# waleedbinkhalid74/cnn-gp

Measured on AMD Instinct MI355X. Metric: kernel entries/s (N×M pairs) + full-Kxx build+solve wall-clock, MNIST 28×28, higher is better.
Workload: dtype f64; 1 GPU; mnist_paper_convnet_gp Kxx 4096x4096, tiles 1024; n=4096, tile=1024, parallelism=tiles-dp1

## Files before the change

### cnn-gp_amd/cnn_gp/_native.py

```python
from __future__ import annotations

import ctypes
import os
import threading

_HERE = os.path.dirname(os.path.abspath(__file__))
LIB_PATH = os.environ.get("CNNGP_LIB",
                          os.path.join(os.path.dirname(_HERE), "lib", "libcnngp.so"))

CGP_ABI_VERSION = 12
CGP_FLAG_EXACT_RELU = 1
CGP_FLAG_GENERIC_CONV = 2
CGP_FLAG_NET_DUAL = 4
CGP_PRE_NONE, CGP_PRE_RELU, CGP_PRE_MOMENTS = 0, 1, 2
CGP_POST_NONE, CGP_POST_RELU = 0, 1
CGP_NET_CONV, CGP_NET_RELU, CGP_NET_MOMENTS, CGP_NET_LINEAR = 0, 1, 2, 3
CGP_NET_LOAD, CGP_NET_STORE = 4, 5
CGP_NET_CODE_HS_CLEAN = 0x100
CGP_NET_CODE_SUM = 0x200
CGP_NET_CODE_FROM_SUM = 0x400
CGP_NET_CODE_GEOMETRY = 0xff
CGP_VAR_MOMENTS, CGP_VAR_CONV, CGP_VAR_HALF, CGP_VAR_SUM = 0, 1, 2, 3

_vp = ctypes.c_void_p
_i64 = ctypes.c_int64
_i32 = ctypes.c_int32
_f64 = ctypes.c_double


class ConvArgs(ctypes.Structure):
    _fields_ = [
        ("in_", _vp), ("in_y", _vp), ("out", _vp), ("addend", _vp),
        ("pre_xx", _vp), ("pre_yy", _vp), ("post_xx", _vp), ("post_yy", _vp),
        ("nmaps", _i64), ("n1", _i64), ("n2", _i64),
        ("h", _i32), ("w", _i32), ("ho", _i32), ("wo", _i32),
        ("taps", _i32), ("offset", _i32), ("stride", _i32), ("dilation", _i32),
        ("channels", _i32), ("pre", _i32), ("post", _i32), ("same", _i32), ("diag", _i32),
        ("maps_per_block", _i32), ("flags", _i32), ("reserved", _i32),
        ("weight", _f64), ("bias", _f64),
    ]


class ReluArgs(ctypes.Structure):
    _fields_ = [
        ("xy", _vp), ("out", _vp), ("addend", _vp), ("xx", _vp), ("yy", _vp),
        ("nmaps", _i64), ("n1", _i64), ("n2", _i64),
        ("hw", _i32), ("same", _i32), ("diag", _i32), ("flags", _i32),
    ]


class ReluNtkArgs(ctypes.Structure):
    _fields_ = [
        ("xy", _vp), ("theta", _vp), ("out_xy", _vp), ("out_theta", _vp),
        ("xx", _vp), ("yy", _vp),
        ("nmaps", _i64), ("n1", _i64), ("n2", _i64),
# ... 23 lines not shown


class VarArgs(ctypes.Structure):
    _fields_ = [
        ("x", _vp), ("y", _vp), ("out", _vp), ("ops", _vp),
        ("n1", _i64), ("n2", _i64), ("store_total", _i64),
        ("nops", _i32), ("channels", _i32), ("h", _i32), ("w", _i32),
        ("lds_elems", _i32), ("scratch", _i32),
    ]


class NetArgs(ctypes.Structure):
    _fields_ = [
        ("x", _vp), ("y", _vp), ("out", _vp), ("kdiag", _vp), ("ops", _vp),
        ("n1", _i64), ("n2", _i64), ("ldo", _i64),
        ("nops", _i32), ("channels", _i32), ("h", _i32), ("w", _i32),
        ("same", _i32), ("final_slot", _i32), ("hs", _i32), ("lds_elems", _i32),
        ("flags", _i32), ("pairs", _i32), ("unit_begin", _i64), ("unit_end", _i64),
        ("final_stage", _i32), ("program", _i32), ("part", _i32),
    ]


def make_fastdiv(d: int):
    s = 0
    while (1 << s) < d:
        s += 1
    m = (((1 << 32) * ((1 << s) - d)) // d + 1) & 0xFFFFFFFF
    return m, s


SIGNATURES = {
    "cgp_abi_version": (_i32, []),
    "cgp_net_xvar_scale": (ctypes.c_double, []),
    "cgp_last_error": (ctypes.c_char_p, []),
    "cgp_conv_args_size": (ctypes.c_size_t, []),
    "cgp_relu_args_size": (ctypes.c_size_t, []),
    "cgp_device_count": (_i32, []),
    "cgp_selftest": (_i32, []),
    "cgp_moments_xy_f64": (_i32, [_vp, _vp, _i64, _i64, _i32, _i32, _i32, _vp, _vp]),
    "cgp_moments_xy_f32": (_i32, [_vp, _vp, _i64, _i64, _i32, _i32, _i32, _vp, _vp]),
    "cgp_moments_var_f64": (_i32, [_vp, _vp, _i64, _i64, _i32, _i32, _vp, _vp, _vp]),
    "cgp_moments_var_f32": (_i32, [_vp, _vp, _i64, _i64, _i32, _i32, _vp, _vp, _vp]),
    "cgp_conv_f64": (_i32, [ctypes.POINTER(ConvArgs), _vp]),
    "cgp_conv_f32": (_i32, [ctypes.POINTER(ConvArgs), _vp]),
    "cgp_relu_f64": (_i32, [ctypes.POINTER(ReluArgs), _vp]),
    "cgp_relu_f32": (_i32, [ctypes.POINTER(ReluArgs), _vp]),
    "cgp_relu_ntk_args_size": (ctypes.c_size_t, []),
    "cgp_relu_ntk_f64": (_i32, [ctypes.POINTER(ReluNtkArgs), _vp]),
    "cgp_relu_ntk_f32": (_i32, [ctypes.POINTER(ReluNtkArgs), _vp]),
    "cgp_var_relu_f64": (_i32, [_vp, _vp, _i64, _i64, _i32, _i32, _vp, _vp, _vp]),
    "cgp_var_relu_f32": (_i32, [_vp, _vp, _i64, _i64, _i32, _i32, _vp, _vp, _vp]),
    "cgp_axpby_f64": (_i32, [_f64, _vp, _f64, _vp, _vp, _i64, _vp]),
    "cgp_axpby_f32": (_i32, [_f64, _vp, _f64, _vp, _vp, _i64, _vp]),
    "cgp_scale_batch_f64": (_i32, [_i32, _vp, _vp, _vp, _f64, _vp]),
    "cgp_cast_f32_f64": (_i32, [_vp, _vp, _i64, _vp]),
    "cgp_transpose_f64": (_i32, [_vp, _i64, _i64, _vp, _vp]),
    "cgp_chol_solve_f64": (_i32, [_vp, _i64, _i64, _vp, _i64, _i64, _f64,
                                  ctypes.POINTER(_i64), _vp]),
    "cgp_chol_last_phases": (_i32, [_vp, ctypes.POINTER(_f64)]),
    "cgp_chol_solve_f64_timed": (_i32, [_vp, _i64, _i64, _vp, _i64, _i64, _f64,
                                        ctypes.POINTER(_i64), ctypes.POINTER(_f64), _vp]),
    "cgp_gemm_f64": (_i32, [_vp, _vp, _vp, _i64, _i64, _i64, _vp]),
    "cgp_sym_mirror_f64": (_i32, [_vp, _i64, _i64, _vp, _vp]),
    "cgp_sym_residual_f64": (_i32, [_vp, _i64, _i64, _vp, _vp, _vp, _i64, _i64, _vp, _vp]),
    "cgp_argmax_rows_f64": (_i32, [_vp, _i64, _i64, _vp, _vp]),
    "cgp_pred_var_f64": (_i32, [_vp, _i64, _i64, _vp, _i64, _i64, _vp, _vp, _vp]),
    "cgp_net_geometry": (_i32, [_i32] * 7),
    "cgp_net_hs_elems": (_i32, [_i32]),
    "cgp_net_supertile": (_i32, []),
    "cgp_net_units": (_i32, [_i32]),
    "cgp_net_resolution": (_i32, [_i32, _i32]),
    "cgp_net_op_size": (ctypes.c_size_t, []),
    "cgp_net_args_size": (ctypes.c_size_t, []),
    "cgp_net_occupancy": (_i32, [_i32, _i32, _i32, _i32]),
    "cgp_net_program": (_i32, [_vp, _i32, _i32, _i32, _i32, _i32]),
    "cgp_net_validate": (_i32, [_vp, _i32, _i32]),
    "cgp_net_static_lds": (_i32, []),
    "cgp_net_f64": (_i32, [ctypes.POINTER(NetArgs), _vp]),
    "cgp_net_f32": (_i32, [ctypes.POINTER(NetArgs), _vp]),
    "cgp_var_op_size": (ctypes.c_size_t, []),
    "cgp_var_args_size": (ctypes.c_size_t, []),
    "cgp_var_chain_f64": (_i32, [ctypes.POINTER(VarArgs), _vp]),
    "cgp_var_chain_f32": (_i32, [ctypes.POINTER(VarArgs), _vp]),
}

_lib = None
_lib_err = None
# ... 54 lines not shown
```

### cnn-gp_amd/cnn_gp/kernels.py

```python
from __future__ import annotations

import os
from typing import Optional

import numpy as np
import torch
import torch.nn as nn

from . import _native as N
from .program import Plan

VAR_CHAIN = os.environ.get("CGP_VAR_CHAIN", "1") != "0"

__all__ = ("NNGPKernel", "Conv2d", "ReLU", "Sequential", "Mixture", "Sum", "resnet_block")


def _stream_handle(device):
    return torch.cuda.current_stream(device).cuda_stream


def _to_device(t: torch.Tensor, device) -> torch.Tensor:
    if t.device != device:
        t = t.to(device, non_blocking=True)
    return t.contiguous()


class _ImageVariances:

    __slots__ = ("images", "var", "qvar", "key")

    def __init__(self, images, var, qvar, key):
        self.images, self.var, self.qvar, self.key = images, var, qvar, key

    def __len__(self):
        return len(self.images)


_GENERATION = [0]


class NNGPKernel(nn.Module):

    def __setattr__(self, name, value):
        _GENERATION[0] += 1
        super().__setattr__(name, value)

    def __delattr__(self, name):
        _GENERATION[0] += 1
        super().__delattr__(name)

    def add_module(self, name, module):
        _GENERATION[0] += 1
        super().add_module(name, module)

    def register_buffer(self, name, tensor, persistent=True):
        _GENERATION[0] += 1
        super().register_buffer(name, tensor, persistent)

    def _apply(self, fn, *args, **kwargs):
        _GENERATION[0] += 1
        out = super()._apply(fn, *args, **kwargs)
        _GENERATION[0] += 1
        return out

    def _plan(self, h: int, w: int) -> Plan:
# ... 146 lines not shown
                                                        N.ptr(var0[:n1]), N.ptr(var0[n1:]),
                                                        stream), "cgp_moments_var")
        var = plan.run_variances(var0[:n1], var0[n1:], n1, n2, same, stream,
                                 need=plan.ntk_need_var())
        nmaps = n1 if diag else n1 * n2
        xy0 = torch.empty((nmaps, h, w), dtype=x.dtype, device=x.device)
        N.check(getattr(lib, f"cgp_moments_xy_{sfx}")(N.ptr(x), N.ptr(y), n1, n2, c, h * w,
                                                       int(diag), N.ptr(xy0), stream),
                "cgp_moments_xy")
        k, th = plan.run_pairs_ntk(xy0, var, n1, n2, same, diag, stream)
        if th is None:
            th = torch.zeros_like(k)
        elif th is k:
            th = k.clone()
        shape = (n1,) if diag else (n1, n2)
        return k.view(shape), th.view(shape)

    def _run(self, x, y, same, diag, stream):
        n1, c, h, w = x.shape
        n2 = y.shape[0]
        plan = self._plan(h, w)
        sfx = Plan._sfx(x.dtype)
        lib = N.load()
        if diag and same and VAR_CHAIN and self._net_plan(plan, x.element_size()) is not None:
            fused = plan.run_variances_fused(x, x, n1, n1, True, stream, {plan.vf})
            if fused is not None:
                return fused[0][plan.vf][0].reshape(n1)
        net = None if diag else self._net_plan(plan, x.element_size())
        if net is not None and VAR_CHAIN:
            rec = net.tile_recipe(plan, x, y, n1, n2, same, plan.flags, stream)
            if rec is not None:
                return rec.run(x, y, stream)
            fused = plan.run_variances_fused(x, y, n1, n2, same, stream, net.need_var,
                                             net.quarter_vars(x.dtype, plan.flags),
                                             views=False)
            if fused is not None:
                var, qvar = fused
                return net.run(x, y, var, n1, n2, same, stream, plan.flags, qvar=qvar)
        var0 = torch.empty((n1 + n2, h, w), dtype=x.dtype, device=x.device)
        N.check(getattr(lib, f"cgp_moments_var_{sfx}")(N.ptr(x), N.ptr(y), n1, n2, c, h * w,
                                                        N.ptr(var0[:n1]), N.ptr(var0[n1:]),
                                                        stream), "cgp_moments_var")
        if net is not None:
            var = plan.run_variances(var0[:n1], var0[n1:], n1, n2, same, stream,
                                     need=net.need_var)
            return net.run(x, y, var, n1, n2, same, stream, plan.flags)
        var = plan.run_variances(var0[:n1], var0[n1:], n1, n2, same, stream)
        xy0 = None
        if not plan.moments_fused:
            nmaps = n1 if diag else n1 * n2
            xy0 = torch.empty((nmaps, h, w), dtype=x.dtype, device=x.device)
            N.check(getattr(lib, f"cgp_moments_xy_{sfx}")(N.ptr(x), N.ptr(y), n1, n2, c, h * w,
                                                           int(diag), N.ptr(xy0), stream),
                    "cgp_moments_xy")
        out = plan.run_pairs(x, y, xy0, var, n1, n2, same, diag, stream)
        if plan.final_hw != (1, 1):
            raise RuntimeError(f"the model's output is {plan.final_hw[0]}x{plan.final_hw[1]}"
                               " per pair, not 1x1: add a final Conv2d covering the map")
        return out.view(n1) if diag else out.view(n1, n2)


    def image_variances(self, x: torch.Tensor, max_bytes: Optional[int] = None):
        if x.device.type != "cuda" or x.dtype not in (torch.float32, torch.float64) or \
                x.dim() != 4 or not VAR_CHAIN:
            return None
        n, _, h, w = x.shape
        plan = self._plan(h, w)
        net = self._net_plan(plan, x.element_size())
        if net is None:
            return None
        quarter = net.quarter_vars(x.dtype, plan.flags)
        chain = plan._var_chain(set(net.need_var), set(quarter) & set(net.need_var), x.device)
        if chain is None:
            return None
        size = n * (chain["total"] + chain["qtotal"]) * x.element_size()
        if max_bytes is None:
            max_bytes = torch.cuda.mem_get_info(x.device)[0] // 4
        if size > max_bytes:
            return None
        x = x.contiguous()
        with torch.cuda.device(x.device):
            fused = plan.run_variances_fused(x, x, n, n, True, _stream_handle(x.device),
                                             net.need_var, quarter)
        if fused is None:
            return None
        var, qvar = fused
        return _ImageVariances(x, {v: xx for v, (xx, _) in var.items()}, dict(qvar),
                               (h, w, x.dtype, plan.flags, self._weights_version()))

    def tile_from_variances(self, vx: "_ImageVariances", i0: int, i1: int,
                            vy: "_ImageVariances", j0: int, j1: int, same: bool,
                            out: Optional[torch.Tensor] = None) -> torch.Tensor:
        if vx.key != vy.key:
            raise ValueError("tile_from_variances: the two image sets were prepared for "
                             "different shapes, dtypes or ReLU modes")
        if same and (vx is not vy or (i0, i1) != (j0, j1)):
            raise ValueError("a diagonal tile takes the same rows of one image set")
        if not (0 <= i0 < i1 <= len(vx) and 0 <= j0 < j1 <= len(vy)):
            raise ValueError(f"tile rows [{i0}, {i1}) x cols [{j0}, {j1}) outside the image "
                             f"sets ({len(vx)}, {len(vy)})")
        h, w, dtype, flags, wver = vx.key
        plan = self._plan(h, w)
        if plan.flags != flags:
            raise ValueError("tile_from_variances: the model's ReLU mode changed since "
                             "image_variances")
        if self._weights_version() != wver:
            raise ValueError("tile_from_variances: a Conv2d weight buffer changed since "
                             "image_variances (bind the image sets again)")
        net = self._net_plan(plan, torch.empty((), dtype=dtype).element_size())
        x, y = vx.images[i0:i1], vy.images[j0:j1]
        var = {v: (m[i0:i1], vy.var[v][j0:j1]) for v, m in vx.var.items()}
        qvar = {v: q[i0:i1] for v, q in vx.qvar.items()}
        with torch.cuda.device(x.device):
            return net.run(x, y, var, i1 - i0, j1 - j0, same, _stream_handle(x.device),
                           flags, out=out, qvar=qvar or None)

    def layers(self):
        return 0


class Conv2d(NNGPKernel):

    def __init__(self, kernel_size, stride=1, padding="same", dilation=1,
                 var_weight=1., var_bias=0., in_channel_multiplier=1,
                 out_channel_multiplier=1):
        super().__init__()
        self.kernel_size = kernel_size
        self.stride = stride
        self.dilation = dilation
        self.var_weight = var_weight
        self.var_bias = var_bias
        self.kernel_has_row_of_zeros = False
        self._padding_arg = padding
        if padding == "same":
            self.padding = dilation * (kernel_size // 2)
            self.kernel_has_row_of_zeros = kernel_size % 2 == 0
        else:
            self.padding = padding
        side = kernel_size + 1 if self.kernel_has_row_of_zeros else kernel_size
        kernel = torch.ones(1, 1, side, side)
        if self.kernel_has_row_of_zeros:
            kernel[:, :, 0, :] = 0.
            kernel[:, :, :, 0] = 0.
        self.register_buffer("kernel", kernel * (self.var_weight / self.kernel_size ** 2))
        self.in_channel_multiplier = in_channel_multiplier
        self.out_channel_multiplier = out_channel_multiplier

    def layers(self):
# ... 86 lines not shown
```

### cnn-gp_amd/cnn_gp/netplan.py

```python
from __future__ import annotations

import collections
import ctypes
import dataclasses
import os
import threading
from typing import Optional

import torch

from . import _native as N
from .program import fuse

ALIGN = 2

TIMING = None

USE_PROGRAMS = os.environ.get("CGP_NET_PROGRAMS", "1") != "0"
FUSE_REDUCE = os.environ.get("CGP_NET_FUSE_REDUCE", "1") != "0"
MAX_LDS_BYTES = 160 * 1024
SMALL_STATE_BYTES = 512 << 20
RECIPE_MAX_BYTES = int(os.environ.get("CGP_RECIPE_MAX_MB", "512")) << 20
RECIPE_SLOTS = 32
RECIPE_TOTAL_BYTES = 4 << 30
# ... 520 lines not shown
            o.dst2 = f.get("dst2", -1)
            o.zero_halo = _zero_code(f.get("zero")) | (_zero_code(f.get("zero2")) << 16)
            if var is None:
                continue
            if v is not None:
                vx, vy = var[v]
                o.var_x, o.var_y = vx.data_ptr(), vy.data_ptr()
            if "var2" in f:
                vx, vy = var[f["var2"]]
                o.var2_x, o.var2_y = vx.data_ptr(), vy.data_ptr()
            if f.get("state") == "in":
                o.var_x = state_in.data_ptr()
            elif f.get("state") == "out":
                o.var_x = state_out.data_ptr()
        return arr

    def chunk_units(self, itemsize: int, units: int, device=None) -> int:
        stride = max(max(st.load_stride, st.store_stride) for st in self.stages)
        chunk = CHUNK_BYTES // (stride * itemsize)
        per_unit = sum(st.load_stride for st in self.stages[1:]) * itemsize
        if device is not None and torch.device(device).type == "cuda" and \
                min(chunk, units) * per_unit > SMALL_STATE_BYTES:
            free = torch.cuda.mem_get_info(device)[0]
            chunk = min(chunk, int(free * STATE_FREE_FRAC) // max(1, per_unit))
        return min(max(64, chunk // 64 * 64), units)

    @staticmethod
    def units(n1: int, n2: int, same: bool) -> int:
        st = N.load().cgp_net_supertile()
        nbi, nbj = -(-n1 // st), -(-n2 // st)
        return (nbi * (nbi + 1) // 2 if same else nbi * nbj) * st * st

    def prepare(self, x, y, var, n1: int, n2: int, same: bool, flags: int = 0,
                out: Optional[torch.Tensor] = None, qvar: Optional[dict] = None):
        sfx = "f64" if x.dtype == torch.float64 else "f32"
        if out is None:
            out = torch.empty((n1, n2), dtype=x.dtype, device=x.device)
        if out.shape != (n1, n2) or out.stride(1) != 1 or out.dtype != x.dtype:
            raise ValueError("out must be an [n1, n2] row-major view of the input dtype")
        units = self.units(n1, n2, same)
        multi = len(self.stages) > 1
        chunk = units
        states = [None] * (len(self.stages) + 1)
        if multi:
            chunk = self.chunk_units(x.element_size(), units, x.device)
            for b in range(1, len(self.stages)):
                states[b] = torch.empty((chunk * self.stages[b].load_stride,),
                                        dtype=x.dtype, device=x.device)
        lib = N.load()
        fn = getattr(lib, f"cgp_net_{sfx}")
        launches = []
        keep = []
        quarters = []
        used = self.quarter_vars(x.dtype, flags)
        if used:
            var = dict(var)
            for v in sorted(used):
                vx, vy = var[v]
                if qvar is not None:
                    var[v] = (qvar[v], vy)
                    continue
                q = torch.empty_like(vx)
                quarters.append((vx, q))
                keep.append(q)
                var[v] = (q, vy)
        tmpls = [self._ops_template(sidx, st, flags, x.element_size())
                 for sidx, st in enumerate(self.stages)]
        offs = [0]
        for t in tmpls:
            offs.append(offs[-1] + len(t[0]))
        host = torch.empty((offs[-1],), dtype=torch.uint8, pin_memory=True)
        hb = host.numpy()
        for sidx, (tmpl, slots, what, _) in enumerate(tmpls):
            ptrs = [var[w[0]][w[1]].data_ptr() if isinstance(w, tuple) else
                    (states[sidx] if w == "in" else states[sidx + 1]).data_ptr()
                    for w in what]
            blk = hb[offs[sidx]:offs[sidx + 1]]
            blk[:] = tmpl
            blk.view("<u8")[slots] = ptrs
        ops_dev = host.to(x.device, non_blocking=True)
        keep.append(ops_dev)
        for sidx, st in enumerate(self.stages):
            program = tmpls[sidx][3]
            a = N.NetArgs()
            a.x, a.y, a.out = x.data_ptr(), y.data_ptr(), out.data_ptr()
            if same:
                a.kdiag = var[self.plan.vf][0].data_ptr()
            a.ops = ops_dev.data_ptr() + offs[sidx]
            a.n1, a.n2, a.ldo = n1, n2, out.stride(0)
            a.nops, a.channels, a.h, a.w = st.n_ops, x.shape[1], x.shape[2], x.shape[3]
            a.same, a.final_slot, a.hs, a.lds_elems = int(same), st.final_slot, 0, st.lds_elems
            a.part = st.part
            a.flags = flags | (N.CGP_FLAG_NET_DUAL if st.dual else 0)
            a.pairs = st.pairs
            a.final_stage = int(st.final)
            a.program = program
            launches.append(a)

        pairs = n1 * (n1 - 1) // 2 if same else n1 * n2

        if quarters:
            xscale = lib.cgp_net_xvar_scale()
            nq = len(quarters)
            q_src = (ctypes.c_void_p * nq)(*[N.ptr(s_) for s_, _ in quarters])
            q_dst = (ctypes.c_void_p * nq)(*[N.ptr(q_) for _, q_ in quarters])
            q_n = (ctypes.c_int64 * nq)(*[s_.numel() for s_, _ in quarters])

        def run_all(stream):
            if quarters:
                N.call("cgp_scale_batch_f64", nq, q_src, q_dst, q_n, xscale, stream)
            for u0 in range(0, units, chunk):
                u1 = min(units, u0 + chunk)
                for a in launches:
                    if multi:
                        a.unit_begin, a.unit_end = u0, u1
                    N.check(fn(ctypes.byref(a), stream), "cgp_net")

        def launch(stream, keep=keep, states=states):
            cur = torch.cuda.current_stream(x.device)
            if stream and stream != cur.cuda_stream:
                ext = torch.cuda.ExternalStream(stream, device=x.device)
                ext.wait_stream(cur)
                for t in keep + [s for s in states if s is not None]:
                    t.record_stream(ext)
            if TIMING is not None:
                st_ = torch.cuda.ExternalStream(stream) if stream else torch.cuda.current_stream()
                e0 = torch.cuda.Event(enable_timing=True)
                e1 = torch.cuda.Event(enable_timing=True)
                e0.record(st_)
                run_all(stream)
                e1.record(st_)
                TIMING.append((e0, e1, pairs))
            else:
                run_all(stream)

        launch.args = launches
        launch.states = states
        return launch, out

    def quarter_vars(self, dtype, flags: int = 0) -> set:
        if dtype != torch.float64 or flags & N.CGP_FLAG_EXACT_RELU:
            return set()
        used = self.__dict__.get("_quarter_used")
        if used is None:
            used = set()
            for st in self.stages:
                used |= {v for _, v in st.records if v is not None}
                used |= {f["var2"] for f, _ in st.records if "var2" in f}
            self.__dict__["_quarter_used"] = used
        return set(used)

    def tile_recipe(self, plan, x, y, n1: int, n2: int, same: bool, flags: int, stream):
        if RECIPE_MAX_BYTES <= 0:
            return None
        key = (n1, n2, bool(same), tuple(x.shape[1:]), x.dtype, x.device, flags, stream)
        lock = self.__dict__.setdefault("_recipe_lock", threading.Lock())
        with lock:
            cache = self.__dict__.setdefault("_recipes", collections.OrderedDict())
            if key in cache:
                cache.move_to_end(key)
                return cache[key]
            rec = TileRecipe.build(self, plan, x, y, n1, n2, same, flags, stream)
            if rec is None:
                return None
            cache[key] = rec
            while len(cache) > RECIPE_SLOTS or (
                    len(cache) > 1 and sum(r.nbytes for r in cache.values()) > RECIPE_TOTAL_BYTES):
                cache.popitem(last=False)
            return rec

    def run(self, x, y, var, n1: int, n2: int, same: bool, stream, flags: int = 0,
            out: Optional[torch.Tensor] = None, qvar: Optional[dict] = None):
        launch, out = self.prepare(x, y, var, n1, n2, same, flags, out, qvar)
        launch(stream)
        return out


class TileRecipe:

    def __init__(self):
        self.lock = threading.Lock()

    @classmethod
    def build(cls, net, plan, x, y, n1, n2, same, flags, stream):
        from .program import DevPtr
        need = set(net.need_var)
        quarter = net.quarter_vars(x.dtype, flags) & need
        chain = plan._var_chain(need, quarter, x.device)
        if chain is None or chain["lds"] * x.element_size() > 64 * 1024 or \
                x.shape[2] * x.shape[3] > 1024:
            return None
        m2 = 0 if same else n2
        n = n1 + m2
        item = x.element_size()
        vbytes = (n * chain["total"] + n1 * chain["qtotal"]) * item
        units = net.units(n1, n2, same)
        sbytes = sum(units * st.load_stride for st in net.stages[1:]) * item
        if vbytes + sbytes > RECIPE_MAX_BYTES:
            return None
        r = cls()
        r.nbytes = vbytes + sbytes
        r.shape = (n1, n2, tuple(x.shape[1:]), x.dtype, x.device)
        r.same = bool(same)
        r.vbuf = torch.empty((vbytes // item,), dtype=x.dtype, device=x.device)
        a = N.VarArgs()
        a.out, a.ops = r.vbuf.data_ptr(), chain["ops"].data_ptr()
        a.n1, a.n2, a.store_total = n1, m2, chain["total"]
        a.nops, a.channels, a.h, a.w = chain["nops"], x.shape[1], x.shape[2], x.shape[3]
        a.lds_elems, a.scratch = chain["lds"], chain["scratch"]
        r.va = a
        r.var_fn = getattr(N.load(), f"cgp_var_chain_{plan._sfx(x.dtype)}")
        r.chain_ops = chain["ops"]
        var, qvar = {}, {}
        shapes = plan.prog.shapes
        for v, off in chain["store"].items():
            ho, wo = shapes[v]
            px = DevPtr(r.vbuf, n * off * item)
            var[v] = (px, px if same else DevPtr(r.vbuf, (n * off + n1 * ho * wo) * item))
        for v, off in chain["qstore"].items():
            qvar[v] = DevPtr(r.vbuf, (n * chain["total"] + n1 * off) * item)
        out = torch.empty((n1, n2), dtype=x.dtype, device=x.device)
        r.launch, _ = net.prepare(x, y, var, n1, n2, same, flags, out, qvar or None)
        r.args = r.launch.args
        return r

    def run(self, x, y, stream):
        n1, n2, _, _, _ = self.shape
        out = torch.empty((n1, n2), dtype=x.dtype, device=x.device)
        xp, yp, op = x.data_ptr(), y.data_ptr(), out.data_ptr()
        with self.lock:
            self.va.x, self.va.y = xp, yp
            N.check(self.var_fn(self.va, stream), "cgp_var_chain")
            for a in self.args:
                a.x, a.y, a.out, a.ldo = xp, yp, op, n2
# ... 3 lines not shown
```

### cnn-gp_amd/csrc/cgp_common.h

```cpp
#pragma once

#include <hip/hip_runtime.h>

#include <string>

#include "cnngp.h"
#include "relu_poly.h"

namespace cgp {

int fail(int code, const char* fmt, ...);
int check_launch(const char* what);
int device_cus();
inline hipStream_t as_stream(void* s) { return reinterpret_cast<hipStream_t>(s); }
inline hipError_t stream_device(hipStream_t s, int* dev) {
    if (s == nullptr) return hipGetDevice(dev);
    hipDevice_t d = 0;
    const hipError_t e = hipStreamGetDevice(s, &d);
    if (e == hipSuccess) *dev = (int)d;
    return e;
}

#define CGP_HIP(call)                                                                  \
    do {                                                                               \
// ... 69 lines not shown
__device__ __forceinline__ float rsqrt_fast(float t) { return __builtin_amdgcn_rsqf(t); }
__device__ __forceinline__ double sqrt_fast(double x) {
    const double r = __builtin_amdgcn_rsq(x);
    const double s0 = x * r;
    return __builtin_fma(0.5 * r, __builtin_fma(-s0, s0, x), s0);
}
__device__ __forceinline__ float sqrt_fast(float x) { return x * __builtin_amdgcn_rsqf(x); }
__device__ __forceinline__ double relu_poly(double x) {
    double r = kReluPolyD[kReluPolyDegD];
#pragma unroll
    for (int k = kReluPolyDegD - 1; k >= 0; --k) r = __builtin_fma(r, x, kReluPolyD[k]);
    return r;
}
__device__ __forceinline__ float relu_poly(float x) {
    float r = kReluPolyF[kReluPolyDegF];
#pragma unroll
    for (int k = kReluPolyDegF - 1; k >= 0; --k) r = __builtin_fmaf(r, x, kReluPolyF[k]);
    return r;
}
__device__ __forceinline__ double fmin_t(double a, double b) { return __builtin_fmin(a, b); }
__device__ __forceinline__ float fmin_t(float a, float b) { return __builtin_fminf(a, b); }
__device__ __forceinline__ double fmax_t(double a, double b) { return __builtin_fmax(a, b); }
__device__ __forceinline__ float fmax_t(float a, float b) { return __builtin_fmaxf(a, b); }
__device__ __forceinline__ double fabs_t(double a) { return __builtin_fabs(a); }
__device__ __forceinline__ float fabs_t(float a) { return __builtin_fabsf(a); }
__device__ __forceinline__ double fma_t(double a, double b, double c) {
    return __builtin_fma(a, b, c);
}
__device__ __forceinline__ float fma_t(float a, float b, float c) {
    return __builtin_fmaf(a, b, c);
}

constexpr double kXVarScale = 0.0625;
constexpr double kPolyQ = 0.125;
constexpr double poly_q(int k) {
    double v = kReluPolyD[k] * kPolyQ;
    for (int n = 0; n < k; ++n) v *= 0.25;
    return v;
}
struct PolyCoef {
    double c[kReluPolyDegD + 1];
};
constexpr PolyCoef poly_coef(bool quartered) {
    PolyCoef t{};
    for (int k = 0; k <= kReluPolyDegD; ++k) t.c[k] = quartered ? poly_q(k) : kReluPolyD[k];
    return t;
}
static __constant__ PolyCoef kReluPolyTabD = poly_coef(false);
static __constant__ PolyCoef kReluPolyTabDq = poly_coef(true);

template <int D>
struct AdaptCoef {
    double c[D + 1];
};
template <int D>
constexpr AdaptCoef<D> adapt_coef(const double (&p)[D + 1]) {
    AdaptCoef<D> t{};
    for (int k = 0; k <= D; ++k) {
        double v = p[k] * kPolyQ;
        for (int n = 0; n < k; ++n) v *= 0.25;
        t.c[k] = v;
    }
    return t;
}
static __constant__ AdaptCoef<kReluAdaptDeg0> kReluAdaptTab0 = adapt_coef<kReluAdaptDeg0>(kReluAdaptP0);
static __constant__ AdaptCoef<kReluAdaptDeg1> kReluAdaptTab1 = adapt_coef<kReluAdaptDeg1>(kReluAdaptP1);
static __constant__ AdaptCoef<kReluAdaptDeg2> kReluAdaptTab2 = adapt_coef<kReluAdaptDeg2>(kReluAdaptP2);
// ... 66 lines not shown
    }
#pragma unroll
    for (int r = 0; r < R; ++r)
        c[r] = __builtin_fma(sx[r], p[r], (c[r] + __builtin_fabs(c[r])) * 0.25);
}
template <int R, int D>
__device__ __forceinline__ void horner_q(double (&p)[R], const double (&u)[R], ConstD t) {
#pragma unroll
    for (int r = 0; r < R; ++r) p[r] = fma_sc(t[D], u[r], t[D - 1]);
#pragma unroll
    for (int k = D - 2; k >= 0; --k) {
        const double ck = t[k];
#pragma unroll
        for (int r = 0; r < R; ++r) p[r] = fma_sc(p[r], u[r], ck);
    }
}
#ifndef CGP_RELU_VOTE_HI
#define CGP_RELU_VOTE_HI 1
#endif
__device__ __forceinline__ unsigned vote_hi(double v) {
    return (unsigned)(__builtin_bit_cast(unsigned long long, v) >> 32);
}
template <int R>
__device__ __forceinline__ unsigned vote_hi_max(const double (&u)[R]) {
    unsigned m = vote_hi(u[0]);
#pragma unroll
    for (int r = 1; r < R; ++r) m = m > vote_hi(u[r]) ? m : vote_hi(u[r]);
    return m;
}
template <int R, bool QIN, int AD = 0>
__device__ __forceinline__ void relu_q_n(double (&c)[R], const double (&v1q)[R],
                                         const double (&v2)[R], const PolyTab& tab,
                                         unsigned long long seg = ~0ull) {
    double y[R], st[R], sx[R], u[R], p[R];
#pragma unroll
    for (int r = 0; r < R; ++r) {
        if constexpr (!QIN) c[r] *= 0.25;
        const double T = __builtin_fma(v1q[r], v2[r], kXVarScale * K<double>::tiny);
        const double r0 = __builtin_amdgcn_rsq(T);
        const double m = T * r0;
        const double k = __builtin_fma(-m, r0, 3.0);
        y[r] = r0 * k;
        st[r] = m * k;
    }
#pragma unroll
    for (int r = 0; r < R; ++r) {
        u[r] = __builtin_fmax(__builtin_fma(-__builtin_fabs(c[r]), y[r], 2.0), 2.0 - 2.0 * kRhoMax);
        const double h = __builtin_amdgcn_rsq(u[r]);
        const double m = u[r] * h;
        const double sq4 = m * __builtin_fma(-m, h, 3.0);
        sx[r] = (st[r] * u[r]) * sq4;
    }
    if constexpr (AD == 2) {
        const unsigned long long ex = __builtin_amdgcn_read_exec() & seg;
        auto all_seg = [&](bool pred) { return (__ballot(pred) & seg) == ex; };
#if CGP_RELU_VOTE_HI
        const unsigned hm = vote_hi_max<R>(u);
        if (all_seg(hm < vote_hi(4.0 * kReluAdaptX0))) {
            horner_q<R, kReluAdaptDeg0>(p, u, tab.a0);
        } else if (all_seg(hm < vote_hi(4.0 * kReluAdaptX1))) {
            horner_q<R, kReluAdaptDeg1>(p, u, tab.a1);
        } else if (all_seg(hm < vote_hi(4.0 * kReluAdaptX2))) {
#else
        double um = u[0];
#pragma unroll
        for (int r = 1; r < R; ++r) um = __builtin_fmax(um, u[r]);
        if (all_seg(um <= 4.0 * kReluAdaptX0)) {
            horner_q<R, kReluAdaptDeg0>(p, u, tab.a0);
        } else if (all_seg(um <= 4.0 * kReluAdaptX1)) {
            horner_q<R, kReluAdaptDeg1>(p, u, tab.a1);
        } else if (all_seg(um <= 4.0 * kReluAdaptX2)) {
#endif
            horner_q<R, kReluAdaptDeg2>(p, u, tab.a2);
        } else {
            horner_q<R, kReluPolyDegD>(p, u, tab.dq);
        }
    } else if constexpr (AD == 1) {
#if CGP_RELU_VOTE_HI
        const unsigned hm = vote_hi_max<R>(u);
        if (__all(hm < vote_hi(4.0 * kReluAdaptX0))) {
            horner_q<R, kReluAdaptDeg0>(p, u, tab.a0);
        } else if (__all(hm < vote_hi(4.0 * kReluAdaptX1))) {
            horner_q<R, kReluAdaptDeg1>(p, u, tab.a1);
        } else if (__all(hm < vote_hi(4.0 * kReluAdaptX2))) {
#else
// ... 141 lines not shown
```

### cnn-gp_amd/csrc/cnngp.hip

```cpp

#include <hip/hip_runtime.h>
#include <rocblas/rocblas.h>
#include <rocsolver/rocsolver.h>

#include <cstdarg>
#include <cstdio>
#include <algorithm>
#include <cstring>
#include <map>
#include <mutex>
#include <string>
#include <vector>

#include "cnngp.h"
#include "cgp_common.h"

namespace cgp {


thread_local std::string g_last_error;

int fail(int code, const char* fmt, ...) {
    char buf[512];
    va_list ap;
// ... 643 lines not shown
        const int px = (int)(f - img * hw);
        const T* src = (is_x ? x : y) + (size_t)img * c * hw + px;
        T acc = src[0] * src[0];
        for (int k = 1; k < c; ++k) acc += src[(size_t)k * hw] * src[(size_t)k * hw];
        (is_x ? xx : yy)[f] = acc / T(c);
    }
}

template <typename T>
__global__ __launch_bounds__(kBlock) void axpby_kernel(T alpha, const T* __restrict__ a, T beta,
                                                       const T* __restrict__ b, T* out,
                                                       long long n) {
    const long long stride = (long long)gridDim.x * kBlock;
    for (long long e = (long long)blockIdx.x * kBlock + threadIdx.x; e < n; e += stride) {
        const T pa = alpha * a[e];
        out[e] = b ? pa + beta * b[e] : pa;
    }
}

constexpr int kScaleBatch = 32;
struct ScaleBatch {
    const double* src[kScaleBatch];
    double* dst[kScaleBatch];
    long long n[kScaleBatch];
};
__global__ __launch_bounds__(kBlock) void scale_batch_kernel(ScaleBatch b, double alpha) {
    const int k = blockIdx.y;
    const double* __restrict__ src = b.src[k];
    double* __restrict__ dst = b.dst[k];
    const long long n = b.n[k];
    const long long stride = (long long)gridDim.x * kBlock;
    for (long long e = (long long)blockIdx.x * kBlock + threadIdx.x; e < n; e += stride)
        dst[e] = alpha * src[e];
}

__global__ __launch_bounds__(kBlock) void cast_kernel(const float* __restrict__ in,
                                                      double* __restrict__ out, long long n) {
    const long long stride = (long long)gridDim.x * kBlock;
    for (long long e = (long long)blockIdx.x * kBlock + threadIdx.x; e < n; e += stride)
        out[e] = (double)in[e];
}

__global__ __launch_bounds__(kBlock) void transpose_kernel(const double* __restrict__ src,
                                                           long long rows, long long cols,
                                                           double* __restrict__ dst) {
    const long long n = rows * cols;
    const long long stride = (long long)gridDim.x * kBlock;
    for (long long e = (long long)blockIdx.x * kBlock + threadIdx.x; e < n; e += stride) {
        const long long r = e / cols, c = e - r * cols;
        dst[c * rows + r] = src[e];
    }
}

__global__ __launch_bounds__(kBlock) void diag_add_kernel(double* k, long long n, long long ld,
                                                          double v) {
    const long long stride = (long long)gridDim.x * kBlock;
    for (long long e = (long long)blockIdx.x * kBlock + threadIdx.x; e < n; e += stride)
        k[e * ld + e] += v;
}

__global__ __launch_bounds__(kBlock) void row_sumsq_sub_kernel(const double* __restrict__ v,
                                                               long long rows, long long cols,
                                                               long long ld,
                                                               const double* d, double* out) {
    __shared__ double part[kBlock];
    for (long long r = blockIdx.x; r < rows; r += gridDim.x) {
// ... 808 lines not shown
}
int cgp_var_relu_f32(const float* xx, const float* yy, int64_t n1, int64_t n2, int32_t hw,
                     int32_t same, float* xo, float* yo, void* stream) {
    return var_relu_impl<float>(xx, yy, n1, n2, hw, same, xo, yo, stream);
}
int cgp_axpby_f64(double alpha, const double* a, double beta, const double* b, double* out,
                  int64_t n, void* stream) {
    return axpby_impl<double>(alpha, a, beta, b, out, n, stream);
}
int cgp_scale_batch_f64(int32_t count, const double* const* src, double* const* dst,
                        const int64_t* n, double alpha, void* stream) {
    if (count < 0 || (count > 0 && (!src || !dst || !n)))
        return fail(CGP_EINVAL, "scale_batch: bad arguments");
    for (int base = 0; base < count; base += kScaleBatch) {
        ScaleBatch b{};
        long long most = 0;
        const int m = count - base < kScaleBatch ? count - base : kScaleBatch;
        for (int k = 0; k < m; ++k) {
            b.src[k] = src[base + k];
            b.dst[k] = dst[base + k];
            b.n[k] = n[base + k];
            if (b.n[k] < 0 || (b.n[k] > 0 && (!b.src[k] || !b.dst[k])))
                return fail(CGP_EINVAL, "scale_batch: buffer %d", base + k);
            if (b.n[k] > most) most = b.n[k];
        }
        if (most == 0) continue;
        hipLaunchKernelGGL(scale_batch_kernel, dim3(grid_for(most), m), dim3(kBlock), 0,
                           as_stream(stream), b, alpha);
        const int rc = check_launch("scale_batch_kernel");
        if (rc != CGP_OK) return rc;
    }
    return CGP_OK;
}
int cgp_axpby_f32(double alpha, const float* a, double beta, const float* b, float* out,
                  int64_t n, void* stream) {
    return axpby_impl<float>(alpha, a, beta, b, out, n, stream);
}

int cgp_cast_f32_f64(const float* in, double* out, int64_t n, void* stream) {
    if (!in || !out || n < 0) return fail(CGP_EINVAL, "cast: bad arguments");
    if (n == 0) return CGP_OK;
    hipLaunchKernelGGL(cast_kernel, dim3(grid_for(n)), dim3(kBlock), 0, as_stream(stream), in,
                       out, (long long)n);
    return check_launch("cast_kernel");
}

int cgp_transpose_f64(const double* src, int64_t rows, int64_t cols, double* dst,
                      void* stream) {
    if (!src || !dst || rows < 0 || cols < 0) return fail(CGP_EINVAL, "transpose: bad args");
    if (rows * cols == 0) return CGP_OK;
    hipLaunchKernelGGL(transpose_kernel, dim3(grid_for(rows * cols)), dim3(kBlock), 0,
                       as_stream(stream), src, (long long)rows, (long long)cols, dst);
    return check_launch("transpose_kernel");
}

int cgp_sym_mirror_f64(double* k, int64_t n, int64_t ldk, double* diag, void* stream) {
    if (!k || !diag || n <= 0 || ldk < n)
        return fail(CGP_EINVAL, "sym_mirror: bad arguments (n=%lld ldk=%lld)", (long long)n,
                    (long long)ldk);
    const long long tiles = (n + kSymT - 1) / kSymT;
    if (tiles > 65535) return fail(CGP_EINVAL, "sym_mirror: n=%lld too large", (long long)n);
    hipLaunchKernelGGL(sym_mirror_kernel, dim3((unsigned)tiles, (unsigned)tiles), dim3(kBlock),
                       0, as_stream(stream), k, (long long)n, (long long)ldk, diag);
    return check_launch("sym_mirror_kernel");
}

// ... 155 lines not shown
```

### cnn-gp_amd/csrc/netfuse.hip

```cpp

#include "cgp_common.h"


#include <map>
#include <mutex>
#include <utility>
#include <algorithm>
#include <climits>

using namespace cgp;

namespace {

constexpr int kNT = 128;
constexpr int kSplit = 2;
template <int NP>
constexpr int kNTof = NP == 2 ? kSplit * kNT : kNT;
template <int NP>
constexpr int kUnitsOf = NP == 2 ? kSplit : NP;
constexpr int kSTL = 3;
constexpr int kST = 1 << kSTL;
constexpr int kEw = 4;

constexpr int pick_r(int lines, int len, int taps, int s, int epi, int nt) {
// ... 1408 lines not shown
    const int prog = a->program;
    if (prog < 0 || prog > kNumProgs)
        return fail(CGP_EINVAL, "net: program %d of %d", prog, kNumProgs);
    if (prog > 0) {
        const ProgInfo& I = kProgs[prog - 1];
        if (I.nops != a->nops || I.pairs != np || I.dual != (du ? 1 : 0) ||
            I.lds_elems != a->lds_elems || !(I.sizes & (int)sizeof(T)))
            return fail(CGP_EINVAL, "net: program %d does not fit this op list", prog);
    }
    return net_launch<T>(p, p.exact != 0, du, np, lds_bytes, prog, stream);
}

}

extern "C" {

int cgp_net_geometry(int32_t h, int32_t w, int32_t ho, int32_t wo, int32_t taps,
                     int32_t stride, int32_t offset) {
    for (int k = 0; k < kNumGeo; ++k) {
        const GeoRow& g = kGeoTable[k];
        if (g.h == h && g.w == w && g.ho == ho && g.wo == wo && g.taps == taps &&
            g.s == stride && g.off == offset)
            return k;
    }
    return -1;
}

int cgp_net_resolution(int32_t h, int32_t w) { return res_index(h, w); }

size_t cgp_net_op_size(void) { return sizeof(cgp_net_op); }
size_t cgp_net_args_size(void) { return sizeof(cgp_net_args); }

int cgp_net_supertile(void) { return kST; }

int cgp_net_units(int32_t pairs) { return net_units(pairs <= 0 ? 1 : pairs); }

int cgp_net_hs_elems(int32_t code) {
    return (code >= 0 && code < kNumGeo) ? kGeoTable[code].hs_elems : -1;
}

int cgp_net_occupancy(int32_t lds_bytes, int32_t f64, int32_t flags, int32_t pairs) {
    if (pairs <= 0) pairs = 1;
    if (lds_bytes <= 0 || (long long)lds_bytes * pairs > 160 * 1024) return 0;
    return f64 ? net_occupancy_for<double>(lds_bytes, flags, pairs)
               : net_occupancy_for<float>(lds_bytes, flags, pairs);
}

int cgp_net_static_lds(void) { return (int)kStaticLds; }

int cgp_net_validate(const cgp_net_op* ops, int32_t nops, int32_t pairs) {
    if (!ops || nops <= 0) return fail(CGP_EINVAL, "net_validate: NULL or empty op list");
    const int np = pairs <= 0 ? 1 : pairs;
    auto geo = [](const cgp_net_op& r) -> const GeoRow* {
        const int g = r.code & CGP_NET_CODE_GEOMETRY;
        return r.kind == CGP_NET_CONV && r.code >= 0 && g < kNumGeo ? &kGeoTable[g] : nullptr;
    };
    for (int k = 0; k < nops; ++k) {
        const cgp_net_op& r = ops[k];
        const bool sum = r.kind == CGP_NET_CONV && r.code >= 0 && (r.code & CGP_NET_CODE_SUM);
        const bool from = r.kind == CGP_NET_CONV && r.code >= 0 && (r.code & CGP_NET_CODE_FROM_SUM);
        if (sum) {
            const GeoRow* g = geo(r);
            const bool point = g && g->taps == 1 && g->off == 0;
            const bool reduce = g && g->ho == 1 && g->wo == 1 && g->off == 0 &&
                                g->taps == g->h && g->taps == g->w;
            if (!g || g->taps <= 3 || point || reduce)
// ... 46 lines not shown
```

### include/cnngp.h

```cpp
#ifndef CNNGP_H
#define CNNGP_H

#include <stddef.h>
#include <stdint.h>

#ifdef __cplusplus
extern "C" {
#endif

#define CGP_ABI_VERSION 12

#define CGP_OK 0
#define CGP_EINVAL 1001
#define CGP_EHIP 1002
#define CGP_EBLAS 1003

#define CGP_PRE_NONE 0
#define CGP_PRE_RELU 1
#define CGP_PRE_MOMENTS 2
#define CGP_POST_NONE 0
#define CGP_POST_RELU 1

#define CGP_FLAG_EXACT_RELU 1
#define CGP_FLAG_GENERIC_CONV 2

int cgp_abi_version(void);
double cgp_net_xvar_scale(void);
const char* cgp_last_error(void);
size_t cgp_conv_args_size(void);
size_t cgp_relu_args_size(void);
int cgp_device_count(void);
int cgp_selftest(void);

int cgp_moments_xy_f64(const double* x, const double* y, int64_t n1, int64_t n2,
                       int32_t c, int32_t hw, int32_t diag, double* xy, void* stream);
int cgp_moments_xy_f32(const float* x, const float* y, int64_t n1, int64_t n2,
                       int32_t c, int32_t hw, int32_t diag, float* xy, void* stream);
int cgp_moments_var_f64(const double* x, const double* y, int64_t n1, int64_t n2,
                        int32_t c, int32_t hw, double* xx, double* yy, void* stream);
int cgp_moments_var_f32(const float* x, const float* y, int64_t n1, int64_t n2,
                        int32_t c, int32_t hw, float* xx, float* yy, void* stream);

typedef struct cgp_conv_args {
    const void* in;
    const void* in_y;
    void* out;
    const void* addend;
    const void* pre_xx;
    const void* pre_yy;
    const void* post_xx;
    const void* post_yy;
    int64_t nmaps;
    int64_t n1, n2;
    int32_t h, w, ho, wo;
    int32_t taps, offset, stride, dilation;
    int32_t channels;
    int32_t pre, post;
    int32_t same, diag;
    int32_t maps_per_block;
    int32_t flags;
// ... 11 lines not shown
    const void* yy;
    int64_t nmaps, n1, n2;
    int32_t hw, same, diag, flags;
} cgp_relu_args;
int cgp_relu_f64(const cgp_relu_args* args, void* stream);
int cgp_relu_f32(const cgp_relu_args* args, void* stream);

typedef struct cgp_relu_ntk_args {
    const void* xy;
    const void* theta;
    void* out_xy;
    void* out_theta;
    const void* xx;
    const void* yy;
    int64_t nmaps, n1, n2;
    int32_t hw, same, diag, flags;
} cgp_relu_ntk_args;
size_t cgp_relu_ntk_args_size(void);
int cgp_relu_ntk_f64(const cgp_relu_ntk_args* args, void* stream);
int cgp_relu_ntk_f32(const cgp_relu_ntk_args* args, void* stream);

int cgp_var_relu_f64(const double* xx, const double* yy, int64_t n1, int64_t n2, int32_t hw,
                     int32_t same, double* xx_out, double* yy_out, void* stream);
int cgp_var_relu_f32(const float* xx, const float* yy, int64_t n1, int64_t n2, int32_t hw,
                     int32_t same, float* xx_out, float* yy_out, void* stream);

int cgp_axpby_f64(double alpha, const double* a, double beta, const double* b, double* out,
                  int64_t n, void* stream);
int cgp_axpby_f32(double alpha, const float* a, double beta, const float* b, float* out,
                  int64_t n, void* stream);

int cgp_scale_batch_f64(int32_t count, const double* const* src, double* const* dst,
                        const int64_t* n, double alpha, void* stream);

int cgp_cast_f32_f64(const float* in, double* out, int64_t n, void* stream);
int cgp_transpose_f64(const double* src, int64_t rows, int64_t cols, double* dst, void* stream);

int cgp_chol_solve_f64(double* k, int64_t n, int64_t ldk, double* bt, int64_t nrhs,
                       int64_t ldb, double jitter, int64_t* info, void* stream);
int cgp_chol_last_phases(void* stream, double* ms);
int cgp_chol_solve_f64_timed(double* k, int64_t n, int64_t ldk, double* bt, int64_t nrhs,
                             int64_t ldb, double jitter, int64_t* info, double* phase_ms,
                             void* stream);
int cgp_sym_mirror_f64(double* k, int64_t n, int64_t ldk, double* diag, void* stream);
int cgp_sym_residual_f64(const double* k, int64_t n, int64_t ldk, const double* diag,
                         const double* x, double* r, int64_t nrhs, int64_t ldx, double* sumsq,
                         void* stream);
int cgp_gemm_f64(const double* a, const double* b, double* c, int64_t m, int64_t n,
                 int64_t kdim, void* stream);
int cgp_pred_var_f64(const double* k, int64_t n, int64_t ldk, double* kxz, int64_t m,
                     int64_t ldz, const double* kz_diag, double* var, void* stream);
int cgp_argmax_rows_f64(const double* a, int64_t rows, int64_t cols, int64_t* out,
                        void* stream);


#define CGP_NET_CONV 0
#define CGP_NET_RELU 1
#define CGP_NET_MOMENTS 2
#define CGP_NET_LINEAR 3
#define CGP_NET_LOAD 4
#define CGP_NET_STORE 5
#define CGP_NET_CODE_HS_CLEAN 0x100
#define CGP_NET_CODE_SUM 0x200
#define CGP_NET_CODE_FROM_SUM 0x400
#define CGP_NET_CODE_GEOMETRY 0xff

// ... 92 lines not shown
```

Before: 109.4 million pairs/s.

## Precompute per-image reciprocal square-root variances to cut ReLU inner-loop work

Switches the ReLU arc-cosine step in the fused network kernel to take precomputed reciprocal square roots of the per-image variances. The pairwise inner loop now needs only one multiply and one rsqrt/Newton step on the product instead of the older scaled form. A new batched rsqrt kernel fills these root buffers once per image set, and the Python planner, recipe sizing and tile path carry the extra buffers through. This adds memory and a small extra launch, and changes numerics slightly (a clamp on Y, a different polynomial scaling).

```diff
diff --git a/cnn-gp_amd/cnn_gp/_native.py b/cnn-gp_amd/cnn_gp/_native.py
--- a/cnn-gp_amd/cnn_gp/_native.py
+++ b/cnn-gp_amd/cnn_gp/_native.py
@@ -21,6 +21,7 @@
 CGP_NET_CODE_FROM_SUM = 0x400
 CGP_NET_CODE_GEOMETRY = 0xff
 CGP_VAR_MOMENTS, CGP_VAR_CONV, CGP_VAR_HALF, CGP_VAR_SUM = 0, 1, 2, 3
+CGP_VAR_FORM_SCALED, CGP_VAR_FORM_RSQRT = 0, 1
 
 _vp = ctypes.c_void_p
 _i64 = ctypes.c_int64
@@ -110,6 +111,7 @@
 SIGNATURES = {
     "cgp_abi_version": (_i32, []),
     "cgp_net_xvar_scale": (ctypes.c_double, []),
+    "cgp_net_var_form": (_i32, []),
     "cgp_last_error": (ctypes.c_char_p, []),
     "cgp_conv_args_size": (ctypes.c_size_t, []),
     "cgp_relu_args_size": (ctypes.c_size_t, []),
@@ -131,6 +133,7 @@
     "cgp_axpby_f64": (_i32, [_f64, _vp, _f64, _vp, _vp, _i64, _vp]),
     "cgp_axpby_f32": (_i32, [_f64, _vp, _f64, _vp, _vp, _i64, _vp]),
     "cgp_scale_batch_f64": (_i32, [_i32, _vp, _vp, _vp, _f64, _vp]),
+    "cgp_rsqrt_batch_f64": (_i32, [_i32, _vp, _vp, _vp, _vp]),
     "cgp_cast_f32_f64": (_i32, [_vp, _vp, _i64, _vp]),
     "cgp_transpose_f64": (_i32, [_vp, _i64, _i64, _vp, _vp]),
     "cgp_chol_solve_f64": (_i32, [_vp, _i64, _i64, _vp, _i64, _i64, _f64,
diff --git a/cnn-gp_amd/cnn_gp/kernels.py b/cnn-gp_amd/cnn_gp/kernels.py
--- a/cnn-gp_amd/cnn_gp/kernels.py
+++ b/cnn-gp_amd/cnn_gp/kernels.py
@@ -1,5 +1,6 @@
 from __future__ import annotations
 
+import ctypes
 import os
 from typing import Optional
 
@@ -27,10 +28,11 @@
 
 class _ImageVariances:
 
-    __slots__ = ("images", "var", "qvar", "key")
-
-    def __init__(self, images, var, qvar, key):
+    __slots__ = ("images", "var", "qvar", "mvar", "key")
+
+    def __init__(self, images, var, qvar, key, mvar=None):
         self.images, self.var, self.qvar, self.key = images, var, qvar, key
+        self.mvar = mvar or {}
 
     def __len__(self):
         return len(self.images)
@@ -243,11 +245,12 @@
             if rec is not None:
                 return rec.run(x, y, stream)
             fused = plan.run_variances_fused(x, y, n1, n2, same, stream, net.need_var,
-                                             net.quarter_vars(x.dtype, plan.flags),
+                                             net.chain_quarter(x.dtype, plan.flags),
                                              views=False)
             if fused is not None:
                 var, qvar = fused
-                return net.run(x, y, var, n1, n2, same, stream, plan.flags, qvar=qvar)
+                return net.run(x, y, var, n1, n2, same, stream, plan.flags,
+                               qvar=qvar or None)
         var0 = torch.empty((n1 + n2, h, w), dtype=x.dtype, device=x.device)
         N.check(getattr(lib, f"cgp_moments_var_{sfx}")(N.ptr(x), N.ptr(y), n1, n2, c, h * w,
                                                         N.ptr(var0[:n1]), N.ptr(var0[n1:]),
@@ -280,24 +283,34 @@
         net = self._net_plan(plan, x.element_size())
         if net is None:
             return None
-        quarter = net.quarter_vars(x.dtype, plan.flags)
+        quarter = net.chain_quarter(x.dtype, plan.flags)
         chain = plan._var_chain(set(net.need_var), set(quarter) & set(net.need_var), x.device)
         if chain is None:
             return None
-        size = n * (chain["total"] + chain["qtotal"]) * x.element_size()
+        roots = net.root_elems(x.dtype, plan.flags)
+        size = n * (chain["total"] + chain["qtotal"] + roots) * x.element_size()
         if max_bytes is None:
             max_bytes = torch.cuda.mem_get_info(x.device)[0] // 4
         if size > max_bytes:
             return None
         x = x.contiguous()
+        mvar = {}
         with torch.cuda.device(x.device):
-            fused = plan.run_variances_fused(x, x, n, n, True, _stream_handle(x.device),
-                                             net.need_var, quarter)
+            stream = _stream_handle(x.device)
+            fused = plan.run_variances_fused(x, x, n, n, True, stream, net.need_var, quarter)
+            if fused is not None and roots:
+                used = sorted(net.quarter_vars(x.dtype, plan.flags))
+                mvar = {v: torch.empty_like(fused[0][v][0]) for v in used}
+                k = len(used)
+                N.call("cgp_rsqrt_batch_f64", k,
+                       (ctypes.c_void_p * k)(*[fused[0][v][0].data_ptr() for v in used]),
+                       (ctypes.c_void_p * k)(*[mvar[v].data_ptr() for v in used]),
+                       (ctypes.c_int64 * k)(*[mvar[v].numel() for v in used]), stream)
         if fused is None:
             return None
         var, qvar = fused
         return _ImageVariances(x, {v: xx for v, (xx, _) in var.items()}, dict(qvar),
-                               (h, w, x.dtype, plan.flags, self._weights_version()))
+                               (h, w, x.dtype, plan.flags, self._weights_version()), mvar)
 
     def tile_from_variances(self, vx: "_ImageVariances", i0: int, i1: int,
                             vy: "_ImageVariances", j0: int, j1: int, same: bool,
@@ -322,9 +335,10 @@
         x, y = vx.images[i0:i1], vy.images[j0:j1]
         var = {v: (m[i0:i1], vy.var[v][j0:j1]) for v, m in vx.var.items()}
         qvar = {v: q[i0:i1] for v, q in vx.qvar.items()}
+        mvar = {v: (m[i0:i1], vy.mvar[v][j0:j1]) for v, m in vx.mvar.items()}
         with torch.cuda.device(x.device):
             return net.run(x, y, var, i1 - i0, j1 - j0, same, _stream_handle(x.device),
-                           flags, out=out, qvar=qvar or None)
+                           flags, out=out, qvar=qvar or None, mvar=mvar or None)
 
     def layers(self):
         return 0
diff --git a/cnn-gp_amd/cnn_gp/netplan.py b/cnn-gp_amd/cnn_gp/netplan.py
--- a/cnn-gp_amd/cnn_gp/netplan.py
+++ b/cnn-gp_amd/cnn_gp/netplan.py
@@ -576,7 +576,8 @@
         return (nbi * (nbi + 1) // 2 if same else nbi * nbj) * st * st
 
     def prepare(self, x, y, var, n1: int, n2: int, same: bool, flags: int = 0,
-                out: Optional[torch.Tensor] = None, qvar: Optional[dict] = None):
+                out: Optional[torch.Tensor] = None, qvar: Optional[dict] = None,
+                mvar: Optional[dict] = None):
         sfx = "f64" if x.dtype == torch.float64 else "f32"
         if out is None:
             out = torch.empty((n1, n2), dtype=x.dtype, device=x.device)
@@ -596,8 +597,28 @@
         launches = []
         keep = []
         quarters = []
+        roots = []
         used = self.quarter_vars(x.dtype, flags)
-        if used:
+        plain = var
+        rsqrt_form = bool(used) and self.var_form() == N.CGP_VAR_FORM_RSQRT
+        if rsqrt_form:
+            var = dict(var)
+            shapes = self.plan.prog.shapes
+            for v in sorted(used):
+                if mvar is not None:
+                    var[v] = mvar[v]
+                    continue
+                vx, vy = var[v]
+                hw = shapes[v][0] * shapes[v][1]
+                mx = torch.empty((n1 * hw,), dtype=x.dtype, device=x.device)
+                roots.append((vx, mx, n1 * hw))
+                my = mx
+                if vy.data_ptr() != vx.data_ptr() or n1 != n2:
+                    my = torch.empty((n2 * hw,), dtype=x.dtype, device=x.device)
+                    roots.append((vy, my, n2 * hw))
+                keep += [mx, my]
+                var[v] = (mx, my)
+        elif used:
             var = dict(var)
             for v in sorted(used):
                 vx, vy = var[v]
@@ -629,7 +650,7 @@
             a = N.NetArgs()
             a.x, a.y, a.out = x.data_ptr(), y.data_ptr(), out.data_ptr()
             if same:
-                a.kdiag = var[self.plan.vf][0].data_ptr()
+                a.kdiag = plain[self.plan.vf][0].data_ptr()
             a.ops = ops_dev.data_ptr() + offs[sidx]
             a.n1, a.n2, a.ldo = n1, n2, out.stride(0)
             a.nops, a.channels, a.h, a.w = st.n_ops, x.shape[1], x.shape[2], x.shape[3]
@@ -649,10 +670,17 @@
             q_src = (ctypes.c_void_p * nq)(*[N.ptr(s_) for s_, _ in quarters])
             q_dst = (ctypes.c_void_p * nq)(*[N.ptr(q_) for _, q_ in quarters])
             q_n = (ctypes.c_int64 * nq)(*[s_.numel() for s_, _ in quarters])
+        if roots:
+            nr = len(roots)
+            r_src = (ctypes.c_void_p * nr)(*[s_.data_ptr() for s_, _, _ in roots])
+            r_dst = (ctypes.c_void_p * nr)(*[m_.data_ptr() for _, m_, _ in roots])
+            r_n = (ctypes.c_int64 * nr)(*[n_ for _, _, n_ in roots])
 
         def run_all(stream):
             if quarters:
                 N.call("cgp_scale_batch_f64", nq, q_src, q_dst, q_n, xscale, stream)
+            if roots:
+                N.call("cgp_rsqrt_batch_f64", nr, r_src, r_dst, r_n, stream)
             for u0 in range(0, units, chunk):
                 u1 = min(units, u0 + chunk)
                 for a in launches:
@@ -693,6 +721,23 @@
                 used |= {f["var2"] for f, _ in st.records if "var2" in f}
             self.__dict__["_quarter_used"] = used
         return set(used)
+
+    @staticmethod
+    def var_form() -> int:
+        return N.load().cgp_net_var_form()
+
+    def chain_quarter(self, dtype, flags: int = 0) -> set:
+        used = self.quarter_vars(dtype, flags)
+        if used and self.var_form() == N.CGP_VAR_FORM_RSQRT:
+            return set()
+        return used
+
+    def root_elems(self, dtype, flags: int = 0) -> int:
+        used = self.quarter_vars(dtype, flags)
+        if not used or self.var_form() != N.CGP_VAR_FORM_RSQRT:
+            return 0
+        shapes = self.plan.prog.shapes
+        return sum(shapes[v][0] * shapes[v][1] for v in used)
 
     def tile_recipe(self, plan, x, y, n1: int, n2: int, same: bool, flags: int, stream):
         if RECIPE_MAX_BYTES <= 0:
@@ -714,8 +759,9 @@
             return rec
 
     def run(self, x, y, var, n1: int, n2: int, same: bool, stream, flags: int = 0,
-            out: Optional[torch.Tensor] = None, qvar: Optional[dict] = None):
-        launch, out = self.prepare(x, y, var, n1, n2, same, flags, out, qvar)
+            out: Optional[torch.Tensor] = None, qvar: Optional[dict] = None,
+            mvar: Optional[dict] = None):
+        launch, out = self.prepare(x, y, var, n1, n2, same, flags, out, qvar, mvar)
         launch(stream)
         return out
 
@@ -729,7 +775,7 @@
     def build(cls, net, plan, x, y, n1, n2, same, flags, stream):
         from .program import DevPtr
         need = set(net.need_var)
-        quarter = net.quarter_vars(x.dtype, flags) & need
+        quarter = net.chain_quarter(x.dtype, flags) & need
         chain = plan._var_chain(need, quarter, x.device)
         if chain is None or chain["lds"] * x.element_size() > 64 * 1024 or \
                 x.shape[2] * x.shape[3] > 1024:
@@ -738,12 +784,13 @@
         n = n1 + m2
         item = x.element_size()
         vbytes = (n * chain["total"] + n1 * chain["qtotal"]) * item
+        mbytes = n * net.root_elems(x.dtype, flags) * item
         units = net.units(n1, n2, same)
         sbytes = sum(units * st.load_stride for st in net.stages[1:]) * item
-        if vbytes + sbytes > RECIPE_MAX_BYTES:
+        if vbytes + mbytes + sbytes > RECIPE_MAX_BYTES:
             return None
         r = cls()
-        r.nbytes = vbytes + sbytes
+        r.nbytes = vbytes + mbytes + sbytes
         r.shape = (n1, n2, tuple(x.shape[1:]), x.dtype, x.device)
         r.same = bool(same)
         r.vbuf = torch.empty((vbytes // item,), dtype=x.dtype, device=x.device)
diff --git a/cnn-gp_amd/csrc/cgp_common.h b/cnn-gp_amd/csrc/cgp_common.h
--- a/cnn-gp_amd/csrc/cgp_common.h
+++ b/cnn-gp_amd/csrc/cgp_common.h
@@ -125,7 +125,13 @@
 }
 
 constexpr double kXVarScale = 0.0625;
-constexpr double kPolyQ = 0.125;
+#ifndef CGP_RELU_ONE_ROOT
+#define CGP_RELU_ONE_ROOT 1
+#endif
+constexpr int kNetVarForm = CGP_RELU_ONE_ROOT ? CGP_VAR_FORM_RSQRT : CGP_VAR_FORM_SCALED;
+constexpr double kPolyQ = CGP_RELU_ONE_ROOT ? 0.5 : 0.125;
+__device__ __forceinline__ double var_rsqrt8(double v) { return 1.0 / __builtin_sqrt(v * 0.125); }
+constexpr double kYMax = 0x1p66;
 constexpr double poly_q(int k) {
     double v = kReluPolyD[k] * kPolyQ;
     for (int n = 0; n < k; ++n) v *= 0.25;
@@ -258,7 +264,25 @@
 __device__ __forceinline__ void relu_q_n(double (&c)[R], const double (&v1q)[R],
                                          const double (&v2)[R], const PolyTab& tab,
                                          unsigned long long seg = ~0ull) {
-    double y[R], st[R], sx[R], u[R], p[R];
+    double sx[R], u[R], p[R];
+#if CGP_RELU_ONE_ROOT
+    double Y[R];
+#pragma unroll
+    for (int r = 0; r < R; ++r) {
+        if constexpr (!QIN) c[r] *= 0.25;
+        Y[r] = __builtin_fmin(v1q[r] * v2[r], kYMax);
+    }
+#pragma unroll
+    for (int r = 0; r < R; ++r) {
+        u[r] = __builtin_fmax(__builtin_fma(-__builtin_fabs(c[r]), Y[r], 2.0), 2.0 - 2.0 * kRhoMax);
+        const double z = (u[r] * Y[r]) * Y[r];
+        const double h = __builtin_amdgcn_rsq(z);
+        const double m = z * h;
+        const double R2 = h * __builtin_fma(-m, h, 3.0);
+        sx[r] = (u[r] * u[r]) * R2;
+    }
+#else
+    double y[R], st[R];
 #pragma unroll
     for (int r = 0; r < R; ++r) {
         if constexpr (!QIN) c[r] *= 0.25;
@@ -277,6 +301,7 @@
         const double sq4 = m * __builtin_fma(-m, h, 3.0);
         sx[r] = (st[r] * u[r]) * sq4;
     }
+#endif
     if constexpr (AD == 2) {
         const unsigned long long ex = __builtin_amdgcn_read_exec() & seg;
         auto all_seg = [&](bool pred) { return (__ballot(pred) & seg) == ex; };
diff --git a/cnn-gp_amd/csrc/cnngp.hip b/cnn-gp_amd/csrc/cnngp.hip
--- a/cnn-gp_amd/csrc/cnngp.hip
+++ b/cnn-gp_amd/csrc/cnngp.hip
@@ -699,6 +699,15 @@
     const long long stride = (long long)gridDim.x * kBlock;
     for (long long e = (long long)blockIdx.x * kBlock + threadIdx.x; e < n; e += stride)
         dst[e] = alpha * src[e];
+}
+__global__ __launch_bounds__(kBlock) void rsqrt_batch_kernel(ScaleBatch b) {
+    const int k = blockIdx.y;
+    const double* __restrict__ src = b.src[k];
+    double* __restrict__ dst = b.dst[k];
+    const long long n = b.n[k];
+    const long long stride = (long long)gridDim.x * kBlock;
+    for (long long e = (long long)blockIdx.x * kBlock + threadIdx.x; e < n; e += stride)
+        dst[e] = var_rsqrt8(src[e]);
 }
 
 __global__ __launch_bounds__(kBlock) void cast_kernel(const float* __restrict__ in,
@@ -1573,6 +1582,31 @@
     }
     return CGP_OK;
 }
+int cgp_rsqrt_batch_f64(int32_t count, const double* const* src, double* const* dst,
+                        const int64_t* n, void* stream) {
+    if (count < 0 || (count > 0 && (!src || !dst || !n)))
+        return fail(CGP_EINVAL, "rsqrt_batch: bad arguments");
+    for (int k = 0; k < count; ++k)
+        if (n[k] < 0 || (n[k] > 0 && (!src[k] || !dst[k])))
+            return fail(CGP_EINVAL, "rsqrt_batch: buffer %d", k);
+    for (int base = 0; base < count; base += kScaleBatch) {
+        ScaleBatch b{};
+        long long most = 0;
+        const int m = count - base < kScaleBatch ? count - base : kScaleBatch;
+        for (int k = 0; k < m; ++k) {
+            b.src[k] = src[base + k];
+            b.dst[k] = dst[base + k];
+            b.n[k] = n[base + k];
+            if (b.n[k] > most) most = b.n[k];
+        }
+        if (most == 0) continue;
+        hipLaunchKernelGGL(rsqrt_batch_kernel, dim3(grid_for(most), m), dim3(kBlock), 0,
+                           as_stream(stream), b);
+        const int rc = check_launch("rsqrt_batch_kernel");
+        if (rc != CGP_OK) return rc;
+    }
+    return CGP_OK;
+}
 int cgp_axpby_f32(double alpha, const float* a, double beta, const float* b, float* out,
                   int64_t n, void* stream) {
     return axpby_impl<float>(alpha, a, beta, b, out, n, stream);
diff --git a/cnn-gp_amd/csrc/netfuse.hip b/cnn-gp_amd/csrc/netfuse.hip
--- a/cnn-gp_amd/csrc/netfuse.hip
+++ b/cnn-gp_amd/csrc/netfuse.hip
@@ -1464,6 +1464,7 @@
 size_t cgp_net_args_size(void) { return sizeof(cgp_net_args); }
 
 int cgp_net_supertile(void) { return kST; }
+int cgp_net_var_form(void) { return kNetVarForm; }
 
 int cgp_net_units(int32_t pairs) { return net_units(pairs <= 0 ? 1 : pairs); }
 
diff --git a/include/cnngp.h b/include/cnngp.h
--- a/include/cnngp.h
+++ b/include/cnngp.h
@@ -26,6 +26,9 @@
 
 int cgp_abi_version(void);
 double cgp_net_xvar_scale(void);
+#define CGP_VAR_FORM_SCALED 0
+#define CGP_VAR_FORM_RSQRT 1
+int cgp_net_var_form(void);
 const char* cgp_last_error(void);
 size_t cgp_conv_args_size(void);
 size_t cgp_relu_args_size(void);
@@ -103,6 +106,8 @@
 
 int cgp_scale_batch_f64(int32_t count, const double* const* src, double* const* dst,
                         const int64_t* n, double alpha, void* stream);
+int cgp_rsqrt_batch_f64(int32_t count, const double* const* src, double* const* dst,
+                        const int64_t* n, void* stream);
 
 int cgp_cast_f32_f64(const float* in, double* out, int64_t n, void* stream);
 int cgp_transpose_f64(const double* src, int64_t rows, int64_t cols, double* dst, void* stream);
```

Result: faster. 116.9 million pairs/s, median of 6 (+6.8%).
